# tllvvv/lz4-sgori

Hardware: AMD Instinct MI355X
Metric: GiB/s compress+decompress (whole node), 64 KiB blocks; ratio delta vs ref (higher is better)
Workload: dtype u8; 1 GPU; Silesia-proxy, 64 KiB independent blocks (16 x 4 KiB bio_vecs, byU16), round trip; blocks_per_gpu=3234, block_bytes=65536, table_type=byU16, bytes_per_gpu=211943424, corpus_multiplier_k=1, parallelism=dp1 (block shards, one corpus per rank)

## Files before the change

lz4-sgori_amd/csrc/lz4e_compress.hip:

```cpp
#include <hip/hip_runtime.h>
#include <stddef.h>
#include <stdint.h>
#include <stdlib.h>

#include <mutex>

#include "lz4e_device.h"
#include "lz4e_gpu.h"
#include "lz4e_order.h"
#include "lz4e_results.h"

namespace lz4e {

namespace {

constexpr uint32_t kTableBytes = 16384;
constexpr uint32_t kStripe = 256;

typedef __attribute__((address_space(1))) uint8_t gu8;
typedef __attribute__((address_space(1))) uint32_t gu32;
typedef __attribute__((address_space(1))) const uint64_t gcu64;

template <int TT>
struct Table {
    uint32_t* lds;
    LZ4E_DEV uint32_t get(uint32_t h) const {
        if constexpr (TT == kByU16) return reinterpret_cast<uint16_t*>(lds)[h];
        else return lds[h];
    }
    LZ4E_DEV void put(uint32_t h, uint32_t v) const {
        if constexpr (TT == kByU16) reinterpret_cast<uint16_t*>(lds)[h] = (uint16_t)v;
        else lds[h] = v;
    }
    LZ4E_DEV uint32_t reread(uint32_t h) const {
        typedef __attribute__((address_space(3))) volatile uint16_t lvu16;
        typedef __attribute__((address_space(3))) volatile uint32_t lvu32;
        if constexpr (TT == kByU16) return ((lvu16*)lds)[h];
        else return ((lvu32*)lds)[h];
    }
};

struct HbmImage {
    ByteBuf buf;
    LZ4E_DEV uint32_t rd8(uint32_t q) const { return buf_ld8(buf, vaddr(q)); }
    LZ4E_DEV uint32_t wld(uint32_t q) const { return buf_ld32(buf, q); }
    LZ4E_DEV void wld9(uint32_t q, uint32_t* o) const {
        o[0] = wld(q - 4);
#pragma unroll
        for (uint32_t i = 0; i < 8; ++i) o[1 + i] = wld(q + 4 * i);
    }
    static constexpr bool kInLds = false;
    LZ4E_DEV uint32_t ld32(uint32_t q) const { return buf_ld32(buf, vaddr(q)); }
    LZ4E_DEV uint64_t ld64(uint32_t q) const {
        const uint32_t v = vaddr(q);
        return ((uint64_t)buf_ld32(buf, v + 4) << 32) | buf_ld32(buf, v);
    }
    LZ4E_DEV uint32_t stripe(uint32_t X, uint32_t lane) const { return ld32(X - 4 + 4 * lane); }
};

struct LdsImage {
    const uint32_t* w;
    uint32_t last;
    LZ4E_DEV uint32_t word(uint32_t i) const { return w[i < last ? i : last]; }
    LZ4E_DEV uint32_t rd8(uint32_t q) const { return (word(q >> 2) >> ((q & 3) * 8)) & 0xFFu; }
    LZ4E_DEV uint32_t ld32(uint32_t q) const {
        const uint32_t i = q >> 2;
        return alignbyte(word(i + 1), word(i), q & 3);
    }
    LZ4E_DEV uint64_t ld64(uint32_t q) const {
        const uint32_t i = q >> 2, r = q & 3;
        const uint32_t w0 = word(i), w1 = word(i + 1), w2 = word(i + 2);
        return ((uint64_t)alignbyte(w2, w1, r) << 32) |
               alignbyte(w1, w0, r);
    }
    LZ4E_DEV uint32_t stripe(uint32_t X, uint32_t lane) const { return ld32(X - 4 + 4 * lane); }
    LZ4E_DEV uint32_t wld(uint32_t q) const { return ld32(q); }
    LZ4E_DEV void wld9(uint32_t q, uint32_t* o) const {
        const uint32_t i0 = (q >> 2) - 1, r = q & 3;
        uint32_t w[10];
#pragma unroll
        for (uint32_t k = 0; k < 10; ++k) w[k] = word(i0 + k);
#pragma unroll
        for (uint32_t k = 0; k < 9; ++k) o[k] = alignbyte(w[k + 1], w[k], r);
    }
    static constexpr bool kInLds = true;
};

struct Stamps {
    uint64_t t, acc[6], t0, r0;
    uint32_t cnt[4];
    LZ4E_DEV void start() {
        t = clock64();
        t0 = t;
        r0 = realtime64();
        for (int i = 0; i < 6; ++i) acc[i] = 0;
        for (int i = 0; i < 4; ++i) cnt[i] = 0;
    }
    LZ4E_DEV void lap(int phase) {
        const uint64_t now = clock64();
        acc[phase] += now - t;
        t = now;
    }
};
enum { kPhSearch, kPhStripe, kPhLit, kPhCount, kPhRematch, kPhTail };

#ifdef LZ4E_TRACE
#define LZ4E_TR(k, a, b)                                                              \
    do {                                                                              \
        if (kStamps && dbg && lane == 0 && trn < (1u << 16)) {                        \
            dbg[kCompressStampWords + 2 * trn] = ((uint64_t)(k) << 56) | (uint64_t)(a); \
            dbg[kCompressStampWords + 1 + 2 * trn] = (uint64_t)(b);                   \
        }                                                                             \
        trn++;                                                                        \
    } while (0)
#else
#define LZ4E_TR(k, a, b) \
    do {                 \
    } while (0)
#endif

template <int TT>
LZ4E_DEV uint32_t hash_val(uint64_t v) {
    if constexpr (TT == kByU32) return hash5(v, 12);
    else return hash4((uint32_t)v, TT == kByU16 ? 13 : 11);
}

LZ4E_DEV uint32_t stripe_mismatch(uint32_t x, uint32_t u0, uint32_t e, uint32_t lane) {
    const uint32_t b = 4 * lane;
    if (b + 4 <= u0) x = 0;
    else if (b < u0) x &= ~0u << (8 * (u0 - b));
    if (b >= e) x |= 1u;
    else if (b + 4 > e) x |= 1u << (8 * (e - b));
    const uint64_t mm = ballot(x != 0);
    if (mm == 0) return kStripe;
    const uint32_t f = ctz64(mm);
    return 4 * f + (uint32_t)__builtin_ctz(lane_val(x, f)) / 8;
}


LZ4E_DEV void st32(gu8* out, uint32_t at, uint32_t v) { *(gu32*)(out + at) = v; }

LZ4E_DEV uint32_t out_ext(gu8* out, uint32_t at, uint32_t rest, uint32_t lane) {
    const uint32_t nff = rest / 255;
    for (uint32_t k = lane; k < nff; k += kWave) out[at + k] = 0xFF;
    if (lane == 0) out[at + nff] = (uint8_t)(rest - nff * 255);
    return nff + 1;
}

template <class IMG>
LZ4E_DEV void out_copy(gu8* out, uint32_t at, const IMG& img, uint32_t from, uint32_t len,
                       uint32_t lane) {
    constexpr uint32_t kChunk = 4 * 4 * kWave;
    constexpr uint32_t kBig = 2 * kChunk;
    uint32_t base = 0;
    for (; base + kBig <= len; base += kBig) {
        uint32_t w[8];
#pragma unroll
        for (int j = 0; j < 8; ++j) w[j] = img.ld32(from + base + 4 * (j * kWave + lane));
#pragma unroll
        for (int j = 0; j < 8; ++j) st32(out, at + base + 4 * (j * kWave + lane), w[j]);
    }
    for (; base < len; base += kChunk) {
        uint32_t w[4];
#pragma unroll
        for (int j = 0; j < 4; ++j) {
            const uint32_t k = base + 4 * (j * kWave + lane);
            w[j] = k < len ? img.ld32(from + k) : 0;
        }
#pragma unroll
        for (int j = 0; j < 4; ++j) {
            const uint32_t k = base + 4 * (j * kWave + lane);
            if (k < len) st32(out, at + k, w[j]);
        }
    }
}

template <class IMG>
LZ4E_DEV void out_copy_exact(gu8* out, uint32_t at, const IMG& img, uint32_t from, uint32_t len,
                             uint32_t lane) {
    const uint32_t whole = len & ~3u;
    out_copy(out, at, img, from, whole, lane);
    if (lane < len - whole) out[at + whole + lane] = (uint8_t)img.rd8(from + whole + lane);
}

template <class IMG>
LZ4E_DEV uint32_t count_from(const IMG& img, uint32_t p, uint32_t c, uint32_t t,
                             uint32_t matchlimit, uint32_t lane) {
    const uint32_t lim = matchlimit - p;
    while (t < lim) {
        const uint32_t si = img.stripe(p + t, lane);
        const uint32_t sb = img.stripe(c + t, lane);
        const uint32_t u = stripe_mismatch(si ^ sb, 4, 4 + lim - t, lane);
        t += u - 4;
        if (u < kStripe) break;
    }
    return t < lim ? t : lim;
}

template <class IMG>
LZ4E_DEV uint32_t back_from(const IMG& img, uint32_t p, uint32_t c, uint32_t room) {
    const uint32_t lane = lane_id();
    for (uint32_t b = 0; b < room; b += kWave) {
        const uint32_t l = b + lane;
        const bool eq = l < room && img.rd8(p - 1 - (l < room ? l : 0)) == img.rd8(c - 1 - (l < room ? l : 0));
        const uint64_t mm = ballot(!eq);
        if (mm) return b + ctz64(mm);
    }
    return room;
}

typedef __attribute__((address_space(1))) uint64_t gu64;
constexpr uint32_t kRecLenBits = 24;
constexpr uint32_t kShortLit = 32;

LZ4E_DEV uint64_t make_record(uint32_t off, uint32_t L, uint32_t ml) {
    return (uint64_t)(off | ((L & 0xFFu) << 16) | ((ml & 0xFFu) << 24)) |
           ((uint64_t)((L >> 8) | ((ml >> 8) << 16)) << 32);
}

LZ4E_DEV void record_seq(gu64* rec, uint32_t& nrec, uint32_t rmask, uint32_t off, uint32_t L, uint32_t ml,
                         uint32_t lane) {
    if (lane == 0) rec[nrec & rmask] = make_record(off, L, ml);
    nrec += 1;
}

template <class IMG>
LZ4E_DEV void flush_step(const IMG& img, gu8* out, uint64_t r, bool act, uint32_t& op, uint32_t& rpos,
                         uint32_t lane) {
    const uint32_t w0 = (uint32_t)r, w1 = (uint32_t)(r >> 32);
    const uint32_t off = w0 & 0xFFFFu;
    const uint32_t L = ((w0 >> 16) & 0xFFu) | ((w1 & 0xFFFFu) << 8);
    const uint32_t ml = (w0 >> 24) | ((w1 >> 16) << 8);
    const uint32_t mc = ml - 4;
    const uint32_t lx = L >= 15 ? (L - 15) / 255 + 1 : 0;
    const uint32_t mx = ml == 0 ? 0 : 2 + (mc >= 15 ? (mc - 15) / 255 + 1 : 0);
    const uint32_t size = act ? 1 + lx + L + mx : 0;
    const uint32_t span = act ? L + ml : 0;
    const uint32_t oe = wave_incl_add(size), pe = wave_incl_add(span);
    const uint32_t o = op + oe - size;
    const uint32_t lo = o + 1 + lx;
    const uint32_t ip = rpos + pe - span;
    uint64_t wide = ballot(act && (L > kShortLit || lx > 1 || mx > 3));
    while (wide) {
        const uint32_t q = ctz64(wide);
        wide &= wide - 1;
        const uint32_t Lq = lane_val(L, q), mlq = lane_val(ml, q), loq = lane_val(lo, q);
        if (Lq >= 15 + 255) out_ext(out, lane_val(o, q) + 1, Lq - 15, lane);
        if (Lq > kShortLit) {
            if (mlq != 0) out_copy(out, loq, img, lane_val(ip, q), Lq, lane);
            else out_copy_exact(out, loq, img, lane_val(ip, q), Lq, lane);
        }
        lockstep();
        if (mlq >= 4 + 15 + 255) out_ext(out, loq + Lq + 2, mlq - 4 - 15, lane);
    }
    lockstep();
    const uint32_t Ls = act && L <= kShortLit ? L : 0, whole = Ls & ~3u;
    uint32_t tail[3], w[kShortLit / 4];
#pragma unroll
    for (uint32_t j = 0; j < 3; ++j) tail[j] = whole + j < Ls ? img.rd8(ip + whole + j) : 0;
#pragma unroll
    for (uint32_t j = 0; j < kShortLit / 4; ++j) w[j] = 4 * j < whole ? img.ld32(ip + 4 * j) : 0;
#pragma unroll
    for (uint32_t j = 0; j < kShortLit / 4; ++j)
        if (4 * j < whole) st32(out, lo + 4 * j, w[j]);
#pragma unroll
    for (uint32_t j = 0; j < 3; ++j)
        if (whole + j < Ls) out[lo + whole + j] = (uint8_t)tail[j];
    if (act) {
        out[o] = (uint8_t)(((L < 15 ? L : 15) << 4) | (ml == 0 ? 0 : (mc < 15 ? mc : 15)));
        if (lx == 1) out[o + 1] = (uint8_t)(L - 15);
        if (ml != 0) {
            out[lo + L] = (uint8_t)off;
            out[lo + L + 1] = (uint8_t)(off >> 8);
            if (mx == 3) out[lo + L + 2] = (uint8_t)(mc - 15);
        }
    }
    op += lane_val(oe, kWave - 1);
    rpos += lane_val(pe, kWave - 1);
}

template <bool kStamps, class IMG>
LZ4E_DEV void flush_records(const IMG& img, gu8* out, const gu64* rec, uint32_t& nrec, uint32_t& op,
                            uint32_t& rpos, Stamps& st, uint32_t lane) {
    wave_fence();
    for (uint32_t base = 0; base < nrec; base += kWave) {
        const bool act = base + lane < nrec;
        const uint64_t r = act ? rec[base + lane] : 0;
        flush_step(img, out, r, act, op, rpos, lane);
    }
    nrec = 0;
    if (kStamps) st.lap(kPhTail);
}

struct FlushLds {
    uint32_t pub, cons, done, abort;
    uint32_t a0, a1, pad[2];
};
constexpr uint32_t kFlushLdsBytes = sizeof(FlushLds);
constexpr uint32_t kPubBatch = kWave;
#ifndef LZ4E_CSPIN_MAX
#define LZ4E_CSPIN_MAX (1u << 23)
#endif
#ifndef LZ4E_CSPIN_PER_BYTE
#define LZ4E_CSPIN_PER_BYTE 128
#endif
constexpr uint32_t kCSpinMax = LZ4E_CSPIN_MAX, kCSpinPerByte = LZ4E_CSPIN_PER_BYTE;
LZ4E_DEV uint32_t flush_spin_max(uint32_t n) { return kCSpinMax + n * kCSpinPerByte; }

LZ4E_DEV uint32_t hs_acquire(uint32_t* p) {
    return uni(__hip_atomic_load(p, __ATOMIC_ACQUIRE, __HIP_MEMORY_SCOPE_WORKGROUP));
}
LZ4E_DEV void hs_release(uint32_t* p, uint32_t v) {
    lockstep();
    __hip_atomic_store(p, v, __ATOMIC_RELEASE, __HIP_MEMORY_SCOPE_WORKGROUP);
}

LZ4E_DEV bool parser_hand_over(FlushLds* S, uint32_t nrec, uint32_t& pubd, uint32_t& cons, uint32_t rlim,
                               uint32_t n) {
    if (nrec - pubd < kPubBatch && nrec - cons <= rlim) return true;
    if (nrec != pubd) {
        stores_done();
        hs_release(&S->pub, nrec);
        pubd = nrec;
    }
    if (nrec - cons <= rlim) return true;
    const uint32_t spin_max = flush_spin_max(n);
    for (uint32_t k = 0;; ++k) {
        const uint32_t c = hs_acquire(&S->cons);
        if (c != cons) {
            cons = c;
            k = 0;
        }
        if (nrec - cons <= rlim) return true;
        if (k >= spin_max || hs_acquire(&S->abort)) {
            hs_release(&S->abort, 1);
            return false;
        }
        __builtin_amdgcn_s_sleep(2);
    }
}

template <class IMG>
LZ4E_DEV void flusher_wave(FlushLds* S, const IMG& img, gu8* out, const gu64* rec, uint32_t nrecords,
                           uint32_t n, uint32_t D, int32_t* retp, uint32_t* auxp, uint32_t b,
                           uint32_t lane) {
    const uint32_t mask = nrecords - 1, rlim = nrecords - kWave;
    const uint32_t spin_max = flush_spin_max(n);
    uint32_t cons = 0, op = 0, rpos = D, seen = 0;
    for (uint32_t k = 0;; ++k) {
        const bool done = hs_acquire(&S->done) != 0;
        const uint32_t pub = hs_acquire(&S->pub);
        const uint32_t avail = pub - cons;
        if (avail >= kWave || (avail != 0 && (avail > rlim || done))) {
            const uint32_t cnt = avail < kWave ? avail : kWave;
            const bool act = lane < cnt;
            const uint64_t r = act ? rec[(cons + lane) & mask] : 0;
            cons += cnt;
            stores_done();
            hs_release(&S->cons, cons);
            flush_step(img, out, r, act, op, rpos, lane);
            seen = pub;
            k = 0;
            continue;
        }
        if (done) break;
        if (pub != seen) {
            seen = pub;
            k = 0;
        }
        if (k >= spin_max || hs_acquire(&S->abort)) {
            hs_release(&S->abort, 1);
            if (lane == 0) retp[b] = kCompressAborted;
            return;
        }
        __builtin_amdgcn_s_sleep(8);
    }
    if (lane == 0) {
        retp[b] = (int32_t)op;
        if (auxp) {
            auxp[2 * (size_t)b] = S->a0;
            auxp[2 * (size_t)b + 1] = S->a1;
        }
    }
}

template <bool kDefer>
LZ4E_DEV void chain_out(gu8* out, uint32_t& op, gu64* rec, uint32_t& nrec, uint32_t rmask, uint64_t evm,
                        uint32_t nev, uint32_t fe, uint32_t d0, uint64_t lanes_below, uint32_t lane) {
    const bool isev = (evm >> lane) & 1;
    if constexpr (kDefer) {
        if (isev) rec[(nrec + popc64(evm & lanes_below)) & rmask] = fe;
        nrec += nev;
    } else {
        const uint32_t ev = push_lane(lane, isev ? popc64(evm & lanes_below) : 63);
        const uint32_t f = shfl(fe, lane < nev ? ev : 0);
        const uint32_t L = (f >> 16) & 0xFF, mc = (f >> 24) - 4;
        const uint32_t hdr = L >= 15 ? 2 : 1;
        const uint32_t size = lane < nev ? hdr + L + 2 + (mc >= 15 ? 1 : 0) : 0;
        const uint32_t o = op + wave_incl_add(size) - size;
        if (lane < nev) {
            out[o] = (uint8_t)(((L < 15 ? L : 15) << 4) | (mc < 15 ? mc : 15));
            if (L >= 15) out[o + 1] = (uint8_t)(L - 15);
            out[o + hdr + L] = (uint8_t)f;
            out[o + hdr + L + 1] = (uint8_t)(f >> 8);
            if (mc >= 15) out[o + hdr + L + 2] = (uint8_t)(mc - 15);
        }
        const uint64_t le = evm & (lane >= 63 ? ~0ull : ((2ull << lane) - 1));
        const uint32_t s = le ? 63 - (uint32_t)__builtin_clzll(le) : 0;
        const uint32_t qi = popc64(evm & ((1ull << s) - 1));
        const uint32_t Lq = shfl(L, qi), dq = shfl(o + hdr, qi);
        if (le && lane - s < Lq) out[dq + lane - s] = (uint8_t)d0;
        op = lane_val(o + size, nev - 1);
    }
}

constexpr uint32_t kFwdW = 8;
constexpr uint32_t kFwd = 4 * kFwdW;
constexpr uint32_t kLong = 1u << 31;
constexpr uint32_t kNoBk = 0xFF;

LZ4E_DEV uint32_t fwd_match(const uint32_t* a, const uint32_t* b, uint32_t lim) {
    uint32_t m = 16;
#pragma unroll
    for (int i = 3; i >= 1; --i) {
        const uint32_t x = a[i] ^ b[i];
        if (x) m = 4 * (uint32_t)i + ((uint32_t)__builtin_ctz(x) >> 3);
    }
    if (m == 16) {
        m = kFwd;
#pragma unroll
        for (int i = (int)kFwdW - 1; i >= 4; --i) {
            const uint32_t x = a[i] ^ b[i];
            if (x) m = 4 * (uint32_t)i + ((uint32_t)__builtin_ctz(x) >> 3);
        }
    }
    if (a[0] != b[0]) return 0;
    if (m >= lim) return lim;
    return m == kFwd ? (kFwd | kLong) : m;
}

LZ4E_DEV uint32_t fwd_match_lane(const uint32_t* dv, uint32_t cl, uint32_t lim, bool active) {
    uint32_t g[4];
#pragma unroll
    for (uint32_t i = 0; i < 4; ++i) g[i] = shfl(dv[i], cl);
    uint32_t m = 16;
#pragma unroll
    for (int i = 3; i >= 1; --i) {
        const uint32_t x = dv[i] ^ g[i];
        if (x) m = 4 * (uint32_t)i + ((uint32_t)__builtin_ctz(x) >> 3);
    }
    const bool eq0 = dv[0] == g[0];
    if (ballot(active && eq0 && m == 16)) {
        uint32_t h[kFwdW - 4];
#pragma unroll
        for (uint32_t i = 0; i < kFwdW - 4; ++i) h[i] = shfl(dv[4 + i], cl);
        if (m == 16) {
            m = kFwd;
#pragma unroll
            for (int i = (int)kFwdW - 1; i >= 4; --i) {
                const uint32_t x = dv[i] ^ h[i - 4];
                if (x) m = 4 * (uint32_t)i + ((uint32_t)__builtin_ctz(x) >> 3);
            }
        }
    }
    if (!eq0) return 0;
    if (m >= lim) return lim;
    return m == kFwd ? (kFwd | kLong) : m;
}

LZ4E_DEV uint32_t back4(uint32_t a, uint32_t b) {
    const uint32_t x = a ^ b;
    return x ? (uint32_t)__builtin_clz(x) >> 3 : 4;
}

LZ4E_DEV uint64_t lane_val64(uint64_t v, uint32_t k) {
    return ((uint64_t)lane_val((uint32_t)(v >> 32), k) << 32) | lane_val((uint32_t)v, k);
}

LZ4E_DEV uint64_t lane_range(uint32_t a, uint32_t b) {
    return (b >= 63 ? ~0ull : ((2ull << b) - 1)) & ~((1ull << a) - 1);
}

struct CResult {
    int32_t ret = 0;
    uint32_t a0 = 0, a1 = 0;
    bool handed = false;
};
#ifndef LZ4E_GENERIC_FROM
#define LZ4E_GENERIC_FROM 48
#endif
constexpr uint32_t kGenericFrom = LZ4E_GENERIC_FROM;

template <int TT, bool kStamps, bool kDefer, bool kTwo, class IMG>
LZ4E_DEV CResult compress_block(const IMG& img, uint32_t* smem, uint32_t n, gu8* out, uint32_t cap,
                                uint64_t* dbg, uint32_t lane, uint32_t D, bool progress_prio, gu64* rec,
                                uint32_t rlim) {
    static_assert(kDefer || !kTwo, "the flusher wave emits records");
    CResult res;
    const uint32_t rmask = kTwo ? rlim + (kWave - 1) : ~0u;
    [[maybe_unused]] FlushLds* const S = reinterpret_cast<FlushLds*>(smem + kTableBytes / 4);
    [[maybe_unused]] uint32_t pubd = 0, cons = 0;
    const Table<TT> T{smem};
    const uint64_t bound = (uint64_t)n + n / 255 + 16;
    const uint32_t capl = (kDefer || cap >= bound) ? 0xFFFFFFFFu : cap;
    uint32_t op = 0, anchor = D, ip = D;
    uint32_t nrec = 0, rpos = D;
    [[maybe_unused]] uint32_t trn = 0;
    Stamps st;
    if (kStamps) st.start();

    if (n >= kMinLength) {
        const uint32_t mflimit = D + n - kMfLimit;
        const uint32_t matchlimit = D + n - kLastLiterals;
        const uint64_t lanes_below = (1ull << lane) - 1;
        if (D != 0) {
            if (lane == 0) T.put(hash_val<TT>(img.ld64(D)), D);
            lockstep();
        }

        auto emit_match = [&](uint32_t tok, uint32_t tokhi, uint32_t off, uint32_t mc) -> bool {
            const uint32_t op_off = op;
            op += 2;
            if ((uint64_t)op + 6 + (mc >> 8) > capl) return false;
            const uint32_t tokb = tokhi | (mc < 15 ? mc : 15);
            const uint32_t e1 = mc - 15;
            const uint32_t e1w = (mc >= 15 && e1 < 255) ? e1 : 0;
            if (lane == 0) {
                if (op_off == tok + 1) {
                    st32(out, tok, tokb | (off << 8) | (e1w << 24));
                } else {
                    out[tok] = (uint8_t)tokb;
                    st32(out, op_off, off | (e1w << 16));
                }
            }
            if (mc >= 15) {
                if (e1 < 255) {
                    op += 1;
                } else {
                    lockstep();
                    op += out_ext(out, op, e1, lane);
                }
            }
            return true;
        };

        bool rmode = false;
        uint32_t e = D + 1;
        uint32_t s = D + 1;
        uint32_t jb = 0;
        uint32_t pf = 0;
        uint32_t prio_next = (n > 16384 && progress_prio) ? D : ~0u;
        uint64_t guess = ~0ull, pprev = ~0ull;
        uint32_t nB = ~0u, ndm1 = 0, ndv[kFwdW];
        auto preload = [&](uint32_t Bn) {
            if (Bn == nB) return;
            nB = Bn;
            uint32_t o[9];
            img.wld9(Bn + lane, o);
            ndm1 = o[0];
#pragma unroll
            for (uint32_t i = 0; i < kFwdW; ++i) ndv[i] = o[1 + i];
        };
        for (;;) {
            if constexpr (kTwo)
                if (!parser_hand_over(S, nrec, pubd, cons, rlim, n)) goto fail;
            if constexpr (kDefer && !kTwo)
                if (nrec > rlim) flush_records<kStamps>(img, out, rec, nrec, op, rpos, st, lane);
            if (e >= prio_next) {
                const uint32_t q = (uint32_t)(((uint64_t)(e - D) * 4) / n);
                prio_next = q >= 4 ? ~0u : D + (uint32_t)(((uint64_t)(q + 1) * n + 3) / 4);
                wave_prio_for(q);
            }
            consume(pf);
            const uint32_t B = rmode ? e - 2 : e;
            const uint32_t p = B + lane;
            const bool valid = p <= mflimit;
            uint32_t dm1, dv[kFwdW];
            if (B == nB) {
                dm1 = ndm1;
#pragma unroll
                for (uint32_t i = 0; i < kFwdW; ++i) dv[i] = ndv[i];
            } else {
                uint32_t o[9];
                img.wld9(p, o);
                dm1 = o[0];
#pragma unroll
                for (uint32_t i = 0; i < kFwdW; ++i) dv[i] = o[1 + i];
            }
            const uint32_t d0 = dv[0];
            const uint32_t h = hash_val<TT>(((uint64_t)dv[1] << 32) | d0);
            uint32_t c0 = 0, rb = p;
            lockstep();
            if (valid) c0 = T.get(h);
            uint32_t em1 = 0, ev[kFwdW];
            if constexpr (!IMG::kInLds) {
                uint32_t o[9];
                img.wld9(c0, o);
                em1 = o[0];
#pragma unroll
                for (uint32_t i = 0; i < kFwdW; ++i) ev[i] = o[1 + i];
            } else {
                ev[0] = img.wld(c0);
            }
            lockstep();
            if (valid) T.put(h, p);
            lockstep();
            if (valid) rb = T.reread(h);
            const uint64_t cm = ballot(rb != p);
            uint64_t same = 0;
            if (cm) {
                const uint64_t vmask = ballot(valid);
                const uint64_t m = match_any6(rb - B) & vmask;
                if (valid && (m & (m - 1))) same = m;
            }
            const uint64_t clash = ballot(same != 0);
            const uint32_t lim = matchlimit - p;
            uint32_t ml = 0, bk = kNoBk;
            {
                const bool dist_ok = (TT == kByU16) || (c0 + kMaxDistance >= p);
                bool full = true;
                if constexpr (IMG::kInLds) {
                    full = ballot(valid && dist_ok && ev[0] == d0) != 0;
                    if (full) {
                        uint32_t o[9];
                        img.wld9(c0, o);
                        em1 = o[0];
#pragma unroll
                        for (uint32_t i = 1; i < kFwdW; ++i) ev[i] = o[1 + i];
                    }
                }
                if (full) {
                    if (valid && dist_ok) ml = fwd_match(dv, ev, lim);
                    if (p >= 4 && c0 >= 4) bk = back4(dm1, em1);
                }
            }
            const uint64_t hitm = ballot(ml != 0);
            uint64_t put = 0;
            bool generic = false;
            auto lanes_match = [&](uint32_t k, uint32_t cl, uint32_t& m, uint32_t& bb) {
                const uint32_t lk = matchlimit - (B + k);
                uint32_t ak[kFwdW], ac[kFwdW];
#pragma unroll
                for (uint32_t i = 0; i < kFwdW; ++i) {
                    ak[i] = lane_val(dv[i], k);
                    ac[i] = lane_val(dv[i], cl);
                }
                m = fwd_match(ak, ac, lk);
                bb = (B + k >= 4 && B + cl >= 4) ? back4(lane_val(dm1, k), lane_val(dm1, cl)) : kNoBk;
            };

            constexpr uint32_t kStop = 0x80;
            const int32_t lvs0 = (int32_t)mflimit - 1 - (int32_t)B;
            const uint64_t inlim0 =
                lvs0 < 0 ? 0 : (lvs0 >= 63 ? ~0ull : ((2ull << (uint32_t)lvs0) - 1));
            const uint64_t srch0 = (lane >= 63 ? 0 : (~0ull << (lane + 1))) & inlim0;
            auto chain_tables = [&](uint32_t vc, uint32_t vm, uint32_t vb, uint32_t& fc,
                                    uint32_t& fe, uint32_t& jv) {
                fc = kStop;
                fe = 0;
                jv = lane;
                const uint64_t ah = ballot(vm != 0) & srch0;
                const uint32_t j = ah ? ctz64(ah) : 64;
                const uint32_t jj = j < 64 ? j : lane;
                const uint32_t mlj = shfl(vm, jj), cj = shfl(vc, jj), bkj = shfl(vb, jj);
                if (valid) {
                    if (vm != 0) {
                        if (!(vm & kLong)) {
                            fc = lane + vm;
                            fe = (p - vc) | (vm << 24);
                        }
                    } else if (j < 64 && !(mlj & kLong) && bkj != kNoBk) {
                        const uint32_t room = j - lane < cj ? j - lane : cj;
                        const uint32_t cu = bkj < room ? bkj : room;
                        if (!(cu == 4 && room > 4)) {
                            fc = j + mlj;
                            fe = (B + j - cj) | ((j - cu - lane) << 16) | ((mlj + cu) << 24);
                            jv = j;
                        }
                    }
                }
            };
            uint32_t fc0 = kStop, fe0 = 0, jv0 = lane;
            bool have0 = false;
            if constexpr (!IMG::kInLds) pf = img.wld(B + 64 + 4 * lane);
            if (kStamps) { st.cnt[0]++; st.lap(kPhSearch); }

            for (;;) {
                if (rmode && capl == 0xFFFFFFFFu && (!IMG::kInLds || (hitm | clash) != 0)) {
                    if (kStamps) st.lap(kPhStripe);
                    const uint32_t ks = e - B;
                    uint32_t k = ks, nev = 0;
                    uint64_t evm = 0, pch = 0;
                    uint32_t fc = kStop, fe = 0, jv = lane;
                    if (ks < 64) {
                        const bool dyn = (clash >> ks) != 0;
                        if (!dyn) {
                            if (!have0) {
                                chain_tables(c0, ml, bk, fc0, fe0, jv0);
                                have0 = true;
                            }
                            fc = fc0;
                            fe = fe0;
                            jv = jv0;
                        }
                        uint64_t Pg = put | (1ull << (ks - 2)) | (1ull << ks) |
                                      (guess & lane_range(ks, 63));
                        constexpr uint32_t kMaxPass = 6;
                        for (uint32_t pass = 0;; ++pass) {
                            if (kStamps) st.cnt[2]++;
                            if (dyn) {
                                const uint64_t pm =
                                    ((clash >> lane) & 1) ? (same & Pg & lanes_below) : 0;
                                const uint32_t cl = pm ? 63 - (uint32_t)__builtin_clzll(pm) : lane;
                                const uint32_t gm1 = shfl(dm1, cl);
                                const uint32_t fm = fwd_match_lane(dv, cl, lim, pm && valid);
                                uint32_t vc = c0, vm = ml, vb = bk;
                                if (pm) {
                                    vc = B + cl;
                                    vm = valid ? fm : 0;
                                    vb = (p >= 4 && B + cl >= 4) ? back4(dm1, gm1) : kNoBk;
                                }
                                chain_tables(vc, vm, vb, fc, fe, jv);
                            }
                            if (kStamps) st.lap(kPhCount);
                            const uint32_t g1 = shfl(fc, fc & 63);
                            const uint32_t J2 = fc < 64 ? g1 : fc;
                            const uint32_t g2 = shfl(fc, J2 & 63), g3 = shfl(J2, J2 & 63);
                            const uint32_t J3 = J2 < 64 ? g2 : J2;
                            const uint32_t J4 = J2 < 64 ? g3 : J2;
                            k = ks;
                            evm = 0;
                            while (k < 64) {
                                const uint32_t x1 = lane_val(fc, k), x2 = lane_val(J2, k);
                                const uint32_t x3 = lane_val(J3, k), x4 = lane_val(J4, k);
                                if (x1 & kStop) break;
                                evm |= 1ull << k;
                                if (x1 >= 64) { k = x1; break; }
                                if (x2 & kStop) { k = x1; break; }
                                evm |= 1ull << x1;
                                if (x2 >= 64) { k = x2; break; }
                                if (x3 & kStop) { k = x2; break; }
                                evm |= 1ull << x2;
                                if (x3 >= 64) { k = x3; break; }
                                if (x4 & kStop) { k = x3; break; }
                                evm |= 1ull << x3;
                                k = x4;
                            }
                            nev = popc64(evm);
                            {
                                const uint64_t eb = evm & lanes_below;
                                const uint32_t lb = eb ? 63 - (uint32_t)__builtin_clzll(eb) : lane;
                                const uint32_t jl = shfl(jv, lb);
                                pch = ballot(eb != 0 && lane <= jl) | evm | (evm >> 2);
                            }
                            if (!dyn) break;
                            const uint64_t Pn = put | pch;
                            const uint64_t U = pch & ~(evm >> 2);
                            const uint64_t mem = same & lanes_below;
                            const uint64_t cg = mem & Pg, cn = mem & Pn;
                            const bool bad = ((U >> lane) & 1) && cg != cn &&
                                             (cg == 0 || cn == 0 ||
                                              __builtin_clzll(cg) != __builtin_clzll(cn));
                            if (!ballot(bad)) break;
                            if (pass + 1 == kMaxPass) {
                                nev = 0;
                                k = ks;
                                pch = 0;
                                break;
                            }
                            Pg = Pn | (k >= 64 ? 0 : lane_range(k, 63));
                        }
                        put |= pch;
                    }
                    if (kStamps) st.lap(kPhLit);
                    if (nev) {
                        chain_out<kDefer>(out, op, rec, nrec, rmask, evm, nev, fe, d0, lanes_below, lane);
                        e = B + k;
                        anchor = e;
                        if (kStamps) { st.cnt[1] += nev; st.cnt[3] += nev << 16; st.lap(kPhTail); }
                        if (e > mflimit) {
                            ip = e;
                            goto last_literals;
                        }
                    }
                }
                if (kStamps && rmode && capl == 0xFFFFFFFFu) { st.cnt[3]++; st.lap(kPhLit); }
                if (rmode) {
                    const uint32_t k = e - B;
                    if (k > 63) break;
                    const uint64_t prior = put | (1ull << (k - 2));
                    uint32_t c, m;
                    if ((clash >> k) & 1) {
                        const uint64_t pm = lane_val64(same, k) & prior & ((1ull << k) - 1);
                        if (pm == 0) {
                            c = lane_val(c0, k);
                            m = lane_val(ml, k);
                        } else {
                            const uint32_t cl = 63 - (uint32_t)__builtin_clzll(pm);
                            c = B + cl;
                            uint32_t bb;
                            lanes_match(k, cl, m, bb);
                        }
                    } else {
                        c = lane_val(c0, k);
                        m = lane_val(ml, k);
                    }
                    put = prior | (1ull << k);
                    if (kStamps) st.lap(kPhCount);
                    if (m == 0) {
                        rmode = false;
                        s = e = e + 1;
                        jb = 0;
                        continue;
                    }
                    uint32_t t = m & ~kLong;
                    if (m & kLong) t = count_from(img, e, c, kFwd, matchlimit, lane);
                    LZ4E_TR(2, e, ((uint64_t)c << 32) | t);
                    if constexpr (kDefer) record_seq(rec, nrec, rmask, e - c, 0, t, lane);
                    else if (!emit_match(op++, 0, e - c, t - 4)) goto fail;
                    if (kStamps) st.cnt[1]++;
                    e += t;
                    anchor = e;
                    if (e > mflimit) {
                        ip = e;
                        goto last_literals;
                    }
                    continue;
                }

                const uint32_t k0 = e - B;
                if (k0 > 63) break;
                const uint32_t kmax = k0 + 64 - jb < 63 ? k0 + 64 - jb : 63;
                const int32_t lvs = (int32_t)mflimit - 1 - (int32_t)B;
                if (lvs < (int32_t)k0) {
                    ip = jb ? e - 1 : s;
                    goto last_literals;
                }
                const uint32_t lastv = (uint32_t)lvs < kmax ? (uint32_t)lvs : kmax;
                const uint64_t rng = lane_range(k0, lastv);
                const uint64_t A = hitm & ~clash & rng;
                uint64_t CL = clash & rng;
                if (A) CL &= (1ull << ctz64(A)) - 1;
                uint32_t hk = 64, c = 0, m = 0, b = kNoBk;
                uint32_t vc = c0, vm = ml, vb = bk;
                if (CL) {
                    const bool isc = (CL >> lane) & 1;
                    const uint64_t prior_l = put | (lane > k0 ? lane_range(k0, lane - 1) : 0);
                    const uint64_t pm = isc ? (same & prior_l & lanes_below) : 0;
                    const uint32_t cl = pm ? 63 - (uint32_t)__builtin_clzll(pm) : lane;
                    const uint32_t gm1 = shfl(dm1, cl);
                    const uint32_t fm = fwd_match_lane(dv, cl, lim, pm != 0);
                    if (pm) {
                        vc = B + cl;
                        vm = fm;
                        vb = (p >= 4 && B + cl >= 4) ? back4(dm1, gm1) : kNoBk;
                    }
                }
                const uint64_t H = ballot((((CL | A) >> lane) & 1) && vm != 0);
                if (H) {
                    hk = ctz64(H);
                    c = lane_val(vc, hk);
                    m = lane_val(vm, hk);
                    b = lane_val(vb, hk);
                }
                if (hk == 64) {
                    put |= rng;
                    jb += lastv - k0 + 1;
                    e = B + lastv + 1;
                    if (lastv < kmax) {
                        ip = B + lastv;
                        goto last_literals;
                    }
                    if (jb > kGenericFrom) {
                        generic = true;
                        break;
                    }
                    continue;
                }
                put |= lane_range(k0, hk);
                if (kStamps) st.lap(kPhStripe);
                const uint32_t q = B + hk;
                const uint32_t room = q - anchor < c ? q - anchor : c;
                uint32_t cu;
                if (b == kNoBk) {
                    cu = back_from(img, q, c, room);
                } else {
                    cu = b < room ? b : room;
                    if (cu == 4 && room > 4) cu += back_from(img, q - 4, c - 4, room - 4);
                }
                const uint32_t ipm = q - cu, cand = c - cu;
                uint32_t t = m & ~kLong;
                if (m & kLong) t = count_from(img, q, c, kFwd, matchlimit, lane);
                t += cu;
                LZ4E_TR(2, ipm, ((uint64_t)cand << 32) | t);
                const uint32_t L = ipm - anchor;
                if constexpr (kDefer) {
                    record_seq(rec, nrec, rmask, ipm - cand, L, t, lane);
                } else {
                    const uint32_t tok = op++;
                    if ((uint64_t)op + L + 8 + L / 255 > capl) goto fail;
                    uint32_t tokhi;
                    if (L >= 15) {
                        tokhi = 0xF0;
                        op += out_ext(out, op, L - 15, lane);
                    } else {
                        tokhi = L << 4;
                    }
                    if (anchor >= B) {
                        const uint32_t r = lane - (anchor - B);
                        if ((r & 3) == 0 && r < L) st32(out, op + r, d0);
                    } else {
                        out_copy(out, op, img, anchor, L, lane);
                    }
                    op += L;
                    lockstep();
                    if (!emit_match(tok, tokhi, ipm - cand, t - 4)) goto fail;
                }
                if (kStamps) { st.cnt[1]++; st.lap(kPhTail); }
                e = ipm + t;
                anchor = e;
                rmode = true;
                if (e > mflimit) {
                    ip = e;
                    goto last_literals;
                }
            }
            if (kStamps) st.lap(kPhStripe);

            if (!generic) preload(rmode ? e - 2 : e);
            if (valid) {
                const uint64_t pg = same & put;
                bool writer;
                uint32_t v;
                if (same == 0) {
                    writer = true;
                    v = (put >> lane) & 1 ? p : c0;
                } else if (pg) {
                    writer = lane == 63 - (uint32_t)__builtin_clzll(pg);
                    v = p;
                } else {
                    writer = lane == ctz64(same);
                    v = c0;
                }
                if (writer) T.put(h, v);
            }
            {
                const uint64_t R = ~7ull;
                const uint32_t mp = popc64((put ^ pprev) & R), mo = popc64(~put & R);
                guess = mp < mo ? put : ~0ull;
                pprev = put;
            }
            if (kStamps) st.lap(kPhRematch);
            if (!generic) continue;

            {
                uint32_t pbase = jb, qh, ch;
                for (;;) {
                    const uint32_t P = pbase + lane;
                    const uint32_t qq = s + (uint32_t)probe_offset(P);
                    const bool pv = (uint64_t)qq + probe_step(P) <= mflimit;
                    const uint64_t vmask = ballot(pv);
                    if (vmask == 0) {
                        ip = s + (uint32_t)probe_offset(pbase - 1);
                        goto last_literals;
                    }
                    const uint32_t q = pv ? qq : s;
                    uint64_t v;
                    if constexpr (TT == kByU32) v = img.ld64(q);
                    else v = img.ld32(q);
                    const uint32_t vq = (uint32_t)v;
                    const uint32_t hq = hash_val<TT>(v);
                    uint32_t g0 = 0, grb = q;
                    lockstep();
                    if (pv) g0 = T.get(hq);
                    lockstep();
                    if (pv) T.put(hq, q);
                    lockstep();
                    if (pv) grb = T.reread(hq);
                    const uint64_t gcm = ballot(grb != q);
                    uint64_t gsame = 0;
                    uint32_t gc = g0;
                    if (gcm) {
                        uint64_t todo = gcm;
                        do {
                            const uint32_t hg = lane_val(hq, ctz64(todo));
                            const uint64_t mm = ballot(pv && hq == hg);
                            if (hq == hg) gsame = mm;
                            todo &= ~mm;
                        } while (todo);
                        const uint64_t below = gsame & lanes_below;
                        const uint32_t qp =
                            shfl(q, below ? 63 - (uint32_t)__builtin_clzll(below) : lane);
                        if (below) gc = qp;
                    }
                    bool hit = false;
                    if (pv) {
                        const bool dist_ok = (TT == kByU16) || (gc + kMaxDistance >= q);
                        hit = dist_ok && img.ld32(gc) == vq;
                    }
                    const uint64_t hm = ballot(hit);
                    const uint32_t klast = hm ? ctz64(hm) : popc64(vmask) - 1;
                    if (pv) {
                        if (gcm == 0) {
                            if (lane > klast) T.put(hq, g0);
                        } else {
                            const uint64_t upto = klast >= 63 ? ~0ull : ((2ull << klast) - 1);
                            if (lane <= klast) {
                                if ((gsame & upto & ~((2ull << lane) - 1)) == 0) T.put(hq, q);
                            } else if ((gsame & upto) == 0) {
                                T.put(hq, g0);
                            }
                        }
                    }
                    if (hm) {
                        qh = lane_val(q, klast);
                        ch = lane_val(gc, klast);
                        break;
                    }
                    if (vmask != ~0ull) {
                        ip = lane_val(q, klast);
                        goto last_literals;
                    }
                    pbase += kWave;
                }
                const uint32_t room = qh - anchor < ch ? qh - anchor : ch;
                const uint32_t cu = back_from(img, qh, ch, room);
                const uint32_t ipm = qh - cu, cand = ch - cu;
                const uint32_t t = count_from(img, qh, ch, 4, matchlimit, lane) + cu;
                LZ4E_TR(2, ipm, ((uint64_t)cand << 32) | t);
                const uint32_t L = ipm - anchor;
                if constexpr (kDefer) {
                    record_seq(rec, nrec, rmask, ipm - cand, L, t, lane);
                } else {
                    const uint32_t tok = op++;
                    if ((uint64_t)op + L + 8 + L / 255 > capl) goto fail;
                    uint32_t tokhi;
                    if (L >= 15) {
                        tokhi = 0xF0;
                        op += out_ext(out, op, L - 15, lane);
                    } else {
                        tokhi = L << 4;
                    }
                    out_copy(out, op, img, anchor, L, lane);
                    op += L;
                    lockstep();
                    if (!emit_match(tok, tokhi, ipm - cand, t - 4)) goto fail;
                }
                if (kStamps) { st.cnt[1]++; st.lap(kPhLit); }
                e = ipm + t;
                anchor = e;
                rmode = true;
                if (e > mflimit) {
                    ip = e;
                    goto last_literals;
                }
            }
        }
    }

last_literals: {
        const uint32_t R = D + n - anchor;
        if constexpr (kTwo) {
            record_seq(rec, nrec, rmask, 0, R, 0, lane);
            if (lane == 0) S->a0 = ip - D;
            if (lane == 0) S->a1 = R;
            stores_done();
            hs_release(&S->pub, nrec);
            hs_release(&S->done, 1);
            res.handed = true;
            return res;
        } else if constexpr (kDefer) {
            record_seq(rec, nrec, rmask, 0, R, 0, lane);
            flush_records<kStamps>(img, out, rec, nrec, op, rpos, st, lane);
        } else {
            if ((uint64_t)op + R + 1 + (R + 240) / 255 > capl) goto fail;
            if (R >= 15) {
                if (lane == 0) out[op] = 0xF0;
                op += 1;
                op += out_ext(out, op, R - 15, lane);
            } else {
                if (lane == 0) out[op] = (uint8_t)(R << 4);
                op += 1;
            }
            out_copy_exact(out, op, img, anchor, R, lane);
            op += R;
        }
        res.ret = (int32_t)op;
        res.a0 = ip - D;
        res.a1 = R;
        if (kStamps) {
            st.lap(kPhTail);
            if (lane == 0 && dbg) {
                for (int i = 0; i < 6; ++i) dbg[i] = st.acc[i];
                dbg[6] = ((uint64_t)st.cnt[1] << 32) | st.cnt[0];
                dbg[7] = ((uint64_t)st.cnt[3] << 32) | st.cnt[2];
                dbg[8] = clock64() - st.t0;
                dbg[9] = realtime64() - st.r0;
            }
        }
        return res;
    }
fail:
    res.ret = kTwo ? kCompressAborted : 0;
    return res;
}

LZ4E_DEV void stage_block(uint32_t* dstw, const uint8_t* src, uint32_t n, uint32_t lane) {
    const uint32_t padded = (n + 3) & ~3u;
    uint8_t* d8 = reinterpret_cast<uint8_t*>(dstw);
    if ((reinterpret_cast<uintptr_t>(src) & 15) == 0) {
        const uint4* g = reinterpret_cast<const uint4*>(src);
        uint4* l = reinterpret_cast<uint4*>(dstw);
        const uint32_t nv = n / 16;
        constexpr uint32_t U = 8;
        const uint32_t nfull = nv / (U * kWave) * (U * kWave);
        for (uint32_t base = 0; base < nfull; base += U * kWave) {
            uint4 v0 = g[base + 0 * kWave + lane], v1 = g[base + 1 * kWave + lane];
            uint4 v2 = g[base + 2 * kWave + lane], v3 = g[base + 3 * kWave + lane];
            uint4 v4 = g[base + 4 * kWave + lane], v5 = g[base + 5 * kWave + lane];
            uint4 v6 = g[base + 6 * kWave + lane], v7 = g[base + 7 * kWave + lane];
            l[base + 0 * kWave + lane] = v0; l[base + 1 * kWave + lane] = v1;
            l[base + 2 * kWave + lane] = v2; l[base + 3 * kWave + lane] = v3;
            l[base + 4 * kWave + lane] = v4; l[base + 5 * kWave + lane] = v5;
            l[base + 6 * kWave + lane] = v6; l[base + 7 * kWave + lane] = v7;
        }
        for (uint32_t i = nfull + lane; i < nv; i += kWave) l[i] = g[i];
        for (uint32_t i = nv * 16 + lane; i < padded; i += kWave) d8[i] = i < n ? src[i] : 0;
    } else {
        for (uint32_t i = lane; i < padded; i += kWave) d8[i] = i < n ? src[i] : 0;
    }
}

template <bool kStamps, bool kDefer, bool kTwo, class IMG>
LZ4E_DEV CResult dispatch_class(const IMG& img, uint32_t* smem, uint32_t n, int tt, gu8* out,
                                uint32_t cap, uint64_t* dbg, uint32_t lane, uint32_t D, bool pp,
                                gu64* rec, uint32_t rlim) {
    if (tt == kByU32)
        return compress_block<kByU32, kStamps, kDefer, kTwo>(img, smem, n, out, cap, dbg, lane, D, pp, rec, rlim);
    if (tt == kByU16)
        return compress_block<kByU16, kStamps, kDefer, kTwo>(img, smem, n, out, cap, dbg, lane, 0, pp, rec, rlim);
    return compress_block<kByU64, kStamps, kDefer, kTwo>(img, smem, n, out, cap, dbg, lane, 0, pp, rec, rlim);
}

template <bool kStamps, bool kRecords, bool kTwo, class IMG>
LZ4E_DEV CResult dispatch_emit(const IMG& img, uint32_t* smem, uint32_t n, int tt, gu8* out,
                               uint32_t cap, uint64_t* dbg, uint32_t lane, uint32_t D, bool pp,
                               uint64_t* records, uint32_t nrecords, uint32_t b) {
    if constexpr (kRecords) {
        const uint64_t bound = (uint64_t)n + n / 255 + 16;
        if (records != nullptr && cap >= bound && n < (1u << kRecLenBits))
            return dispatch_class<kStamps, true, kTwo>(img, smem, n, tt, out, cap, dbg, lane, D, pp,
                                                 (gu64*)(records + (size_t)b * nrecords), nrecords - kWave);
    }
    return dispatch_class<kStamps, false, false>(img, smem, n, tt, out, cap, dbg, lane, D, pp, nullptr, 0);
}

struct CompressArgs {
    const uint8_t* src;
    const uint64_t* src_off;
    const uint32_t* src_len;
    const uint8_t* table_type;
    uint8_t* dst;
    const uint64_t* dst_off;
    const uint32_t* dst_cap;
    int32_t* ret;
    uint32_t* aux;
    uint32_t nblocks;
    uint32_t max_len;
    uint64_t* dbg;
    const uint32_t* dict_len;
    const uint32_t* order;
    uint64_t* records;
    uint32_t nrecords;
};
static_assert(offsetof(CompressArgs, ret) == 56 && offsetof(CompressArgs, order) == 96 &&
                  offsetof(CompressArgs, nrecords) == 112,
              "kernarg layout");

template <bool kLdsInput, bool kStamps, bool kRecords>
constexpr bool kTwoWave = !kLdsInput && kRecords && !kStamps;

template <bool kLdsInput, bool kStamps, bool kRecords>
__global__ __launch_bounds__((kTwoWave<kLdsInput, kStamps, kRecords> ? 2 : 1) * kWave) void compress_kernel(const uint8_t* __restrict__ src,
                                                      const uint64_t* __restrict__ src_off,
                                                      const uint32_t* __restrict__ src_len,
                                                      const uint8_t* __restrict__ table_type,
                                                      uint8_t* __restrict__ dst,
                                                      const uint64_t* __restrict__ dst_off,
                                                      const uint32_t* __restrict__ dst_cap,
                                                      int32_t* __restrict__ ret,
                                                      uint32_t* __restrict__ aux, uint32_t nblocks,
                                                      uint32_t max_len, uint64_t* __restrict__ dbg,
                                                      const uint32_t* __restrict__ dict_len,
                                                      const uint32_t* __restrict__ order,
                                                      uint64_t* records, uint32_t nrecords) {
    extern __shared__ __attribute__((aligned(16))) uint32_t smem[];
    if (blockIdx.x >= nblocks) return;
    constexpr bool kTwo = kTwoWave<kLdsInput, kStamps, kRecords>;
    constexpr uint32_t kThreads = (kTwo ? 2 : 1) * kWave;
    const uint32_t wave = kTwo ? uni(threadIdx.x / kWave) : 0;
    const uint32_t b = order ? order[blockIdx.x] : blockIdx.x;
    const uint32_t lane = lane_id();
    const uint32_t n = src_len[b];
    const int tt = table_type[b];
    const uint32_t cap = dst_cap[b];
    gu8* out = (gu8*)(dst + dst_off[b]);
    const uint8_t* in = src + src_off[b];
    uint64_t* dbg_slot = dbg ? dbg + kCompressStampWords * (size_t)b : nullptr;

    const uint32_t D = dict_len && dict_len[b] >= 8 ? dict_len[b] : 0;
    const bool tt_ok = (tt == kByU16 && n <= 65536) || tt == kByU32 || tt == kByU64;
    const bool dict_ok = D == 0 || (tt == kByU32 && D <= 65536 && !kLdsInput);
    const bool fits = !kLdsInput || n <= max_len;
    if (n > kMaxInput || (n >= kMinLength && !tt_ok) || !fits || !dict_ok) {
        if (lane == 0 && wave == 0) ret[b] = n > kMaxInput ? 0 : -1;
        return;
    }

    CResult res;
    if (n >= kMinLength) {
        uint4* t4 = reinterpret_cast<uint4*>(smem);
        for (uint32_t i = wave * kWave + lane; i < kTableBytes / 16; i += kThreads) t4[i] = make_uint4(0, 0, 0, 0);
    }
    if constexpr (kTwo) {
        if (wave == 1 && lane < 4) smem[kTableBytes / 4 + lane] = 0;
    }

    if constexpr (kLdsInput) {
        uint32_t* inw = smem + kTableBytes / 4;
        stage_block(inw, in, n, lane);
        block_sync();
        const LdsImage img{inw, n == 0 ? 0 : (n - 1) >> 2};
        res = dispatch_emit<kStamps, kRecords, false>(img, smem, n, tt, out, cap, dbg_slot, lane, 0, true, records,
                                               nrecords, b);
    } else {
        block_sync();
        const uint8_t* base = in - D;
        const HbmImage img{buf_make(base, D + n)};
        if (D != 0 && n >= kMinLength) {
            if (wave == 0)
                for (uint32_t p = 3 * lane; p + 8 <= D; p += 3 * kWave)
                    atomicMax(&smem[hash_val<kByU32>(img.ld64(p))], p);
            block_sync();
        }
        if constexpr (kTwo) {
            if (wave == 1) {
                const uint64_t bound = (uint64_t)n + n / 255 + 16;
                if (records != nullptr && cap >= bound && n < (1u << kRecLenBits))
                    flusher_wave((FlushLds*)(smem + kTableBytes / 4), img, out,
                                 (const gu64*)(records + (size_t)b * nrecords), nrecords, n, D, ret, aux, b,
                                 lane);
                return;
            }
        }
        bool pp = true;
        if (order) {
            const uint32_t nh = order[nblocks];
            if (nh < nblocks - nblocks / 16) {
                pp = false;
                if (blockIdx.x < nh) __builtin_amdgcn_s_setprio(3);
            }
        }
        res = dispatch_emit<kStamps, kRecords, kTwo>(img, smem, n, tt, out, cap, dbg_slot, lane, D, pp, records,
                                               nrecords, b);
    }
    if (res.handed) return;
#ifndef LZ4E_EMU
    const __attribute__((address_space(4))) CompressArgs* ka =
        (const __attribute__((address_space(4))) CompressArgs*)__builtin_amdgcn_kernarg_segment_ptr();
    asm volatile("" : "+s"(ka));
    int32_t* const retp = ka->ret;
    uint32_t* const auxp = ka->aux;
    const uint32_t* const ordp = ka->order;
#else
    int32_t* const retp = ret;
    uint32_t* const auxp = aux;
    const uint32_t* const ordp = order;
#endif
    const uint32_t b2 = ordp ? ordp[blockIdx.x] : blockIdx.x;
    if (lane == 0) {
        retp[b2] = res.ret;
        if (auxp) {
            auxp[2 * (size_t)b2] = res.a0;
            auxp[2 * (size_t)b2 + 1] = res.a1;
        }
    }
}

constexpr uint32_t kWeightChunks = 16, kWeightChunk = 256, kWeightThreads = 256;
constexpr uint32_t kOrderMinBlocks = 1024;
constexpr uint32_t kOrderMinLen = 16384;

__global__ __launch_bounds__(kWeightThreads) void weight_kernel(const uint8_t* __restrict__ src,
                                                                const uint64_t* __restrict__ src_off,
                                                                const uint32_t* __restrict__ src_len,
                                                                uint32_t nblocks,
                                                                uint32_t* __restrict__ weight) {
    constexpr uint32_t kPer = kWeightChunks * kWeightChunk / kWeightThreads;
    constexpr uint32_t kTab = 256;
    __shared__ __attribute__((aligned(16))) uint8_t smp[kWeightChunks * kWeightChunk + 16];
    __shared__ uint32_t hist[256], cnt[2], tbl[kWeightChunks * kTab];
    __shared__ float esum;
    const uint32_t b = blockIdx.x, t = threadIdx.x;
    if (b >= nblocks) return;
    const uint32_t n = src_len[b];
    if (n < kWeightChunk * 2) {
        if (t == 0) weight[b] = 0;
        return;
    }
    const uint8_t* in = src + src_off[b];
    const uint32_t c = t / (kWeightChunk / kPer), r0 = (t % (kWeightChunk / kPer)) * kPer;
    const uint32_t base = (uint32_t)((uint64_t)(n - kWeightChunk) * c / (kWeightChunks - 1));
    hist[t] = 0;
    if (t < 2) cnt[t] = 0;
    if (t == 0) esum = 0.f;
    for (uint32_t i = t; i < kWeightChunks * kTab; i += kWeightThreads) tbl[i] = ~0u;
#pragma unroll
    for (uint32_t k = 0; k < kPer; ++k) smp[c * kWeightChunk + r0 + k] = in[base + r0 + k];
    if (t < 16) smp[kWeightChunks * kWeightChunk + t] = 0;
    __syncthreads();
    const uint8_t* ch = smp + c * kWeightChunk;
    const uint32_t* chw = (const uint32_t*)ch;
    uint32_t* tb = tbl + c * kTab;
    uint32_t d[kPer / 4 + 1];
#pragma unroll
    for (uint32_t i = 0; i <= kPer / 4; ++i) d[i] = chw[r0 / 4 + i];
    const uint32_t prev = r0 ? ch[r0 - 1] : 0x100u;
    auto word_at = [&](uint32_t r) -> uint32_t {
        return alignbyte(chw[r / 4 + 1], chw[r / 4], r & 3);
    };
    uint32_t w[kPer];
    uint32_t runs = 0;
#pragma unroll
    for (uint32_t k = 0; k < kPer; ++k) {
        const uint32_t r = r0 + k;
        w[k] = alignbyte(d[k / 4 + 1], d[k / 4], k & 3);
        if (k % 4 == 0) atomicAdd(&hist[w[k] & 0xFFu], 1u);
        const uint32_t pb = k == 0 ? prev : (d[(k - 1) / 4] >> (8 * ((k - 1) & 3))) & 0xFFu;
        if (r + 4 <= kWeightChunk) {
            tb[(w[k] * 2654435761u) >> 24] = r;
            runs += w[k] == pb * 0x01010101u;
        }
    }
    __syncthreads();
    uint32_t seen = 0;
#pragma unroll
    for (uint32_t k = 0; k < kPer; ++k) {
        const uint32_t r = r0 + k;
        if (r + 4 <= kWeightChunk) {
            const uint32_t f = tb[(w[k] * 2654435761u) >> 24];
            seen += f != r && word_at(f) == w[k];
        }
    }
    {
        const uint32_t rs = wave_incl_add(runs), ss = wave_incl_add(seen);
        if ((t & 63) == 63) {
            atomicAdd(&cnt[0], rs);
            atomicAdd(&cnt[1], ss);
        }
    }
    const float p = (float)hist[t] / (float)(kWeightChunks * kWeightChunk / 4);
    if (p > 0.f) atomicAdd(&esum, -p * log2f(p));
    __syncthreads();
    if (t == 0) {
        const float npos = (float)(kWeightChunks * (kWeightChunk - 3));
        const float R = (float)cnt[0] / npos, S = (float)cnt[1] / npos;
        weight[b] = esum > 7.5f ? 0u : (uint32_t)(1000.f * (1.f - R) * (0.2f + S));
    }
}

struct CompressWeight {
    const uint32_t* weight;
    LZ4E_DEV uint32_t operator()(uint32_t b) const {
        const uint32_t q = weight[b] * (kOrderBuckets - 1) / 1200;
        return (kOrderBuckets - 1) - (q < kOrderBuckets - 1 ? q : kOrderBuckets - 1);
    }
};
constexpr uint32_t kHeavyBucket = kOrderBuckets - 1 - 7;

uint32_t env_u32(const char* name, uint32_t dflt) {
    const char* e = getenv(name);
    return e ? (uint32_t)strtoul(e, nullptr, 10) : dflt;
}

constexpr uint32_t kRecMin = kWave, kRecMax = 4096, kRecDefault = 1024;
constexpr size_t kRecBudget = (size_t)64 << 20;
uint32_t record_slots(uint32_t nblocks) {
    const char* e = getenv("LZ4E_COMPRESS_RECORDS");
    const uint32_t want = e ? (uint32_t)strtoul(e, nullptr, 10) : kRecDefault;
    if (want == 0) return 0;
    uint32_t r = kRecMin;
    while (2 * r <= want && 2 * r <= kRecMax) r *= 2;
    while (r > kRecMin && sizeof(uint64_t) * (size_t)nblocks * r > kRecBudget) r /= 2;
    return sizeof(uint64_t) * (size_t)nblocks * r <= kRecBudget ? r : 0;
}
#ifndef LZ4E_EMU
hipError_t launch_alloc(void** p, size_t bytes, hipStream_t stream) {
    constexpr int kMaxDevices = 64;
    static std::mutex mu;
    static hipMemPool_t pools[kMaxDevices];
    static bool tried[kMaxDevices];
    int dev = -1;
    hipMemPool_t pool = nullptr;
    if (hipGetDevice(&dev) == hipSuccess && dev >= 0 && dev < kMaxDevices) {
        std::lock_guard<std::mutex> lk(mu);
        if (!tried[dev]) {
            tried[dev] = true;
            hipMemPoolProps props = {};
            props.allocType = hipMemAllocationTypePinned;
            props.handleTypes = hipMemHandleTypeNone;
            props.location.type = hipMemLocationTypeDevice;
            props.location.id = dev;
            uint64_t keep = kRecBudget + ((uint64_t)1 << 20);
            if (hipMemPoolCreate(&pools[dev], &props) != hipSuccess ||
                hipMemPoolSetAttribute(pools[dev], hipMemPoolAttrReleaseThreshold, &keep) != hipSuccess) {
                (void)hipGetLastError();
                pools[dev] = nullptr;
            }
        }
        pool = pools[dev];
    }
    if (pool != nullptr && hipMallocFromPoolAsync(p, bytes, pool, stream) == hipSuccess) return hipSuccess;
    (void)hipGetLastError();
    return hipMallocAsync(p, bytes, stream);
}
#else
hipError_t launch_alloc(void** p, size_t bytes, hipStream_t stream) { return hipMallocAsync(p, bytes, stream); }
#endif

#ifdef LZ4E_EMU
constexpr bool kDeferLds = true;
#else
constexpr bool kDeferLds = false;
#endif

template <bool kStamps>
hipError_t launch_compress_impl(const CompressBatch& a, hipStream_t stream, uint64_t* dbg) {
    if (a.nblocks == 0) return hipSuccess;
    static const uint32_t lds_max = env_u32("LZ4E_COMPRESS_LDS_MAX", kMaxLdsInput);
    const bool lds_input = a.max_len <= lds_max && a.dict_len == nullptr;
    const dim3 grid(a.nblocks), block(kWave);
    uint32_t lds = compress_lds_bytes(a.max_len, lds_input);
    constexpr bool kTwo = kTwoWave<false, kStamps, true>;
    if (kTwo && !lds_input) lds += kFlushLdsBytes;
    const int om = launch_order_mode(true);
    const bool use_order = !lds_input && (om == kOrderAlways || (om == kOrderAuto && a.nblocks >= kOrderMinBlocks &&
                                                                 a.max_len >= kOrderMinLen));
    const uint32_t nrec = (!lds_input || kDeferLds) ? record_slots(a.nblocks) : 0;
    const size_t rec_bytes = sizeof(uint64_t) * (size_t)a.nblocks * nrec;
    const size_t order_bytes = use_order ? sizeof(uint32_t) * (2 * (size_t)a.nblocks + 1) : 0;
    uint8_t* pool = nullptr;
    if (rec_bytes + order_bytes != 0 &&
        launch_alloc((void**)&pool, rec_bytes + order_bytes, stream) != hipSuccess) {
        (void)hipGetLastError();
        pool = nullptr;
    }
    uint64_t* records = pool && nrec ? (uint64_t*)pool : nullptr;
    uint32_t* scratch = pool && use_order ? (uint32_t*)(pool + rec_bytes) : nullptr;
    if (lds_input) {
        hipLaunchKernelGGL((compress_kernel<true, kStamps, kDeferLds>), grid, block, lds, stream, a.src,
                           a.src_off, a.src_len, a.table_type, a.dst, a.dst_off, a.dst_cap, a.ret,
                           a.aux, a.nblocks, a.max_len, dbg, a.dict_len, nullptr, records, nrec);
    } else {
        if (scratch) {
            hipLaunchKernelGGL(weight_kernel, dim3(a.nblocks), dim3(kWeightThreads), 0, stream, a.src,
                               a.src_off, a.src_len, a.nblocks, scratch);
            hipLaunchKernelGGL((order_kernel<CompressWeight>), dim3(1), dim3(kOrderThreads), 0, stream,
                               CompressWeight{scratch}, a.nblocks, scratch + a.nblocks, kHeavyBucket,
                               scratch + 2 * (size_t)a.nblocks);
        }
        hipLaunchKernelGGL((compress_kernel<false, kStamps, true>), grid, dim3((kTwo ? 2 : 1) * kWave), lds, stream, a.src,
                           a.src_off, a.src_len, a.table_type, a.dst, a.dst_off, a.dst_cap, a.ret,
                           a.aux, a.nblocks, a.max_len, dbg, a.dict_len,
                           scratch ? (const uint32_t*)(scratch + a.nblocks) : nullptr, records, nrec);
    }
    const hipError_t err = hipGetLastError();
    if (pool) (void)hipFreeAsync(pool, stream);
    return err;
}

}

uint32_t compress_lds_bytes(uint32_t max_len, bool lds_input) {
    uint32_t bytes = kTableBytes;
    if (lds_input) bytes += (max_len + 15) & ~15u;
    return bytes;
}

hipError_t launch_compress(const CompressBatch& a, hipStream_t stream) {
    return launch_compress_impl<false>(a, stream, nullptr);
}

hipError_t launch_compress_stamped(const CompressBatch& a, hipStream_t stream, uint64_t* dbg) {
    return launch_compress_impl<true>(a, stream, dbg);
}

}
```

Baseline: 51.27 GiB/s.

## Group clashing lanes via LDS atomics and flatten event chain-walk loop

Result: faster. 52.68 GiB/s (median of 6 runs) (+2.7%).

```diff
diff --git a/lz4-sgori_amd/csrc/lz4e_compress.hip b/lz4-sgori_amd/csrc/lz4e_compress.hip
--- a/lz4-sgori_amd/csrc/lz4e_compress.hip
+++ b/lz4-sgori_amd/csrc/lz4e_compress.hip
@@ -15,6 +15,10 @@
 namespace {
 
 constexpr uint32_t kTableBytes = 16384;
+constexpr uint32_t kStageOff = kTableBytes;
+constexpr uint32_t kFlushLdsOff = kTableBytes;
+constexpr uint32_t kGroupLdsOff = kFlushLdsOff + 32;
+constexpr uint32_t kGroupLdsBytes = 64 * sizeof(uint64_t);
 constexpr uint32_t kStripe = 256;
 
 typedef __attribute__((address_space(1))) uint8_t gu8;
@@ -297,6 +301,7 @@
     uint32_t a0, a1, pad[2];
 };
 constexpr uint32_t kFlushLdsBytes = sizeof(FlushLds);
+static_assert(kFlushLdsOff + kFlushLdsBytes == kGroupLdsOff, "the slots follow the hand-over");
 constexpr uint32_t kPubBatch = kWave;
 #ifndef LZ4E_CSPIN_MAX
 #define LZ4E_CSPIN_MAX (1u << 23)
@@ -414,6 +419,15 @@
     }
 }
 
+LZ4E_DEV uint64_t group_lanes(uint64_t* slot, uint32_t key, uint32_t lane) {
+    uint64_t* const mine = slot + (key & (kWave - 1));
+    if (key == lane) slot[lane] = 0;
+    lockstep();
+    __hip_atomic_fetch_or(mine, 1ull << lane, __ATOMIC_RELAXED, __HIP_MEMORY_SCOPE_WAVEFRONT);
+    lockstep();
+    return *mine;
+}
+
 constexpr uint32_t kFwdW = 8;
 constexpr uint32_t kFwd = 4 * kFwdW;
 constexpr uint32_t kLong = 1u << 31;
@@ -498,7 +512,8 @@
     static_assert(kDefer || !kTwo, "the flusher wave emits records");
     CResult res;
     const uint32_t rmask = kTwo ? rlim + (kWave - 1) : ~0u;
-    [[maybe_unused]] FlushLds* const S = reinterpret_cast<FlushLds*>(smem + kTableBytes / 4);
+    [[maybe_unused]] FlushLds* const S = reinterpret_cast<FlushLds*>(smem + kFlushLdsOff / 4);
+    [[maybe_unused]] uint64_t* const X = reinterpret_cast<uint64_t*>(smem + kGroupLdsOff / 4);
     [[maybe_unused]] uint32_t pubd = 0, cons = 0;
     const Table<TT> T{smem};
     const uint64_t bound = (uint64_t)n + n / 255 + 16;
@@ -609,8 +624,9 @@
             const uint64_t cm = ballot(rb != p);
             uint64_t same = 0;
             if (cm) {
-                const uint64_t vmask = ballot(valid);
-                const uint64_t m = match_any6(rb - B) & vmask;
+                uint64_t m;
+                if constexpr (IMG::kInLds) m = match_any6(rb - B) & ballot(valid);
+                else m = group_lanes(X, rb - B, lane);
                 if (valid && (m & (m - 1))) same = m;
             }
             const uint64_t clash = ballot(same != 0);
@@ -723,29 +739,38 @@
                                 chain_tables(vc, vm, vb, fc, fe, jv);
                             }
                             if (kStamps) st.lap(kPhCount);
+                            constexpr uint32_t kEnd = kStop << 1;
+                            auto flagged = [](uint32_t j, uint32_t nxt) {
+                                return j | (((j | (nxt & kStop)) + 0xC0) & kEnd);
+                            };
                             const uint32_t g1 = shfl(fc, fc & 63);
                             const uint32_t J2 = fc < 64 ? g1 : fc;
                             const uint32_t g2 = shfl(fc, J2 & 63), g3 = shfl(J2, J2 & 63);
                             const uint32_t J3 = J2 < 64 ? g2 : J2;
                             const uint32_t J4 = J2 < 64 ? g3 : J2;
+                            const uint32_t g4 = shfl(fc, J4 & 63);
+                            const uint32_t F1 = flagged(fc, g1), F2 = flagged(J2, g2);
+                            const uint32_t F3 = flagged(J3, J4), F4 = flagged(J4, g4);
                             k = ks;
                             evm = 0;
-                            while (k < 64) {
-                                const uint32_t x1 = lane_val(fc, k), x2 = lane_val(J2, k);
-                                const uint32_t x3 = lane_val(J3, k), x4 = lane_val(J4, k);
-                                if (x1 & kStop) break;
-                                evm |= 1ull << k;
-                                if (x1 >= 64) { k = x1; break; }
-                                if (x2 & kStop) { k = x1; break; }
-                                evm |= 1ull << x1;
-                                if (x2 >= 64) { k = x2; break; }
-                                if (x3 & kStop) { k = x2; break; }
-                                evm |= 1ull << x2;
-                                if (x3 >= 64) { k = x3; break; }
-                                if (x4 & kStop) { k = x3; break; }
-                                evm |= 1ull << x3;
-                                k = x4;
-                            }
+                            if (!(lane_val(fc, ks) & kStop))
+                                for (;;) {
+                                    const uint32_t x1 = lane_val(F1, k), x2 = lane_val(F2, k);
+                                    const uint32_t x3 = lane_val(F3, k), x4 = lane_val(F4, k);
+                                    evm |= 1ull << k;
+                                    k = x1;
+                                    if (x1 & kEnd) break;
+                                    evm |= 1ull << x1;
+                                    k = x2;
+                                    if (x2 & kEnd) break;
+                                    evm |= 1ull << x2;
+                                    k = x3;
+                                    if (x3 & kEnd) break;
+                                    evm |= 1ull << x3;
+                                    k = x4;
+                                    if (x4 & kEnd) break;
+                                }
+                            k &= kStop - 1;
                             nev = popc64(evm);
                             {
                                 const uint64_t eb = evm & lanes_below;
@@ -1223,11 +1248,11 @@
         for (uint32_t i = wave * kWave + lane; i < kTableBytes / 16; i += kThreads) t4[i] = make_uint4(0, 0, 0, 0);
     }
     if constexpr (kTwo) {
-        if (wave == 1 && lane < 4) smem[kTableBytes / 4 + lane] = 0;
+        if (wave == 1 && lane < 4) smem[kFlushLdsOff / 4 + lane] = 0;
     }
 
     if constexpr (kLdsInput) {
-        uint32_t* inw = smem + kTableBytes / 4;
+        uint32_t* inw = smem + kStageOff / 4;
         stage_block(inw, in, n, lane);
         block_sync();
         const LdsImage img{inw, n == 0 ? 0 : (n - 1) >> 2};
@@ -1247,7 +1272,7 @@
             if (wave == 1) {
                 const uint64_t bound = (uint64_t)n + n / 255 + 16;
                 if (records != nullptr && cap >= bound && n < (1u << kRecLenBits))
-                    flusher_wave((FlushLds*)(smem + kTableBytes / 4), img, out,
+                    flusher_wave((FlushLds*)(smem + kFlushLdsOff / 4), img, out,
                                  (const gu64*)(records + (size_t)b * nrecords), nrecords, n, D, ret, aux, b,
                                  lane);
                 return;
@@ -1442,7 +1467,7 @@
     const dim3 grid(a.nblocks), block(kWave);
     uint32_t lds = compress_lds_bytes(a.max_len, lds_input);
     constexpr bool kTwo = kTwoWave<false, kStamps, true>;
-    if (kTwo && !lds_input) lds += kFlushLdsBytes;
+    if (!lds_input) lds += kFlushLdsBytes + kGroupLdsBytes;
     const int om = launch_order_mode(true);
     const bool use_order = !lds_input && (om == kOrderAlways || (om == kOrderAuto && a.nblocks >= kOrderMinBlocks &&
                                                                  a.max_len >= kOrderMinLen));
```
